# aticejiang/MLAgg-UNet

Measured on AMD Instinct MI355X. Metric: images/sec (train step) MLAgg-UNet-2D 256x256 bs10, higher is better.
Workload: dtype f32; 1 GPU; nnUNetTrainer_MLAgg_2D_dt_MS train step, AbdomenMRI-shaped 256x256x1, 14 classes, attention variant B (BASELINE.json configs[1]); batch_per_gpu=10, global_batch=10, parallelism=dp1, launch=eager, miopen=tuned find-db (mlagg-unet_amd/miopen_db), library_gemm=TunableOp table (mlagg-unet_amd/gemm_db), tuning off

## Files before the change

include/mlagg_hip.h:

```cpp
#ifndef MLAGG_HIP_H
#define MLAGG_HIP_H

#include <stddef.h>

#ifdef __cplusplus
extern "C" {
#endif

#define MLAGG_E_UNSUPPORTED (-1)
#define MLAGG_E_NULLPTR     (-2)
#define MLAGG_E_WORKSPACE   (-3)

#define MLAGG_DTYPE_F32  0
#define MLAGG_DTYPE_BF16 1
#define MLAGG_DTYPE_F16  2
#define MLAGG_DTYPE_BF16X3 3

const char *mlagg_version(void);
const char *mlagg_error_string(int code);

int mlagg_profile_kernel_count(void);
const char *mlagg_profile_kernel_name(int id);
int mlagg_profile_select(int id);
int mlagg_profile_collect(double *ms, int *counts);
// ... 45 lines not shown
                          float *dlam, float *dsubln_w, float *workspace,
                          int batch, int N, int P, int nh, float scale, void *stream);

int mlagg_dwconv3x3_fwd(const float *x, int x_stride, const float *w, const float *bias, const float *res, float *y,
                        int y_stride, float *pre, int batch, int H, int W, int C, int silu, void *stream);
size_t mlagg_dwconv3x3_bwd_workspace_floats(int batch, int H, int W, int C);
int mlagg_dwconv3x3_gated_fwd(const float *x, int x_stride, const float *w, const float *bias, const float *gate, int gate_stride, float *y,
                              int y_stride, float *pre, int batch, int H, int W, int C, void *stream);
int mlagg_dwconv3x3_gated_bwd(const float *x, int x_stride, const float *w, const float *dy, int dy_stride, const float *pre,
                              const float *gate, int gate_stride, float *dx, int dx_stride, float *dgate, int dgate_stride, float *dw,
                              float *dbias, float *workspace, int batch, int H, int W, int C, void *stream);
int mlagg_dwconv3x3_bwd(const float *x, int x_stride, const float *w, const float *dy, int dy_stride,
                        const float *pre, float *dx, int dx_stride, float *dw, float *dbias, float *workspace,
                        int batch, int H, int W, int C, int silu, void *stream);

int mlagg_linear_fwd(const float *x, int x_stride, const float *w, const float *bias, float *y, int y_stride,
                     int M, int N, int K, void *stream);
int mlagg_linear_dgrad(const float *dy, int dy_stride, const float *w, float *dx, int dx_stride, int M, int O, int I,
                       void *stream);
int mlagg_linear_lp_fwd(const float *x, int x_stride, const float *w, const float *bias, float *y, int y_stride,
                        int M, int N, int K, int dtype, void *stream);
int mlagg_linear_lp_dgrad(const float *dy, int dy_stride, const float *w, float *dx, int dx_stride, int M, int O, int I,
                          int dtype, void *stream);
size_t mlagg_linear_wgrad_workspace_floats(int M, int O, int I);
int mlagg_linear_wgrad(const float *dy, int dy_stride, const float *x, int x_stride, float *dW, float *db,
                       float *workspace, int M, int O, int I, void *stream);
int mlagg_linear_wgrad_x3(const float *dy, int dy_stride, const float *x, int x_stride, float *dW, float *db, float *workspace,
                          int M, int O, int I, void *stream);

int mlagg_flash_attn_fwd(const void *q, const void *k, const void *v, void *out, float *lse, int B, int N, int P, int nh,
                         int head_dim, float softmax_scale, int dtype, void *stream);
size_t mlagg_flash_attn_bwd_workspace_floats(int B, int N, int P, int nh, int head_dim);
int mlagg_flash_attn_bwd(const void *q, const void *k, const void *v, const void *out, const void *dout, const float *lse,
                         void *dq, float *workspace, int B, int N, int P, int nh, int head_dim, float softmax_scale,
                         int dtype, void *stream);

int mlagg_layernorm_supported(int C);
int mlagg_layernorm_fwd(const float *x, int x_stride, const float *gamma, const float *beta, float *y,
                        float *stats, int rows, int C, float eps, void *stream);
size_t mlagg_layernorm_bwd_workspace_floats(int rows, int C);
int mlagg_layernorm_bwd(const float *x, int x_stride, const float *dy, int dy_stride, const float *gamma,
                        const float *stats, float *dx, float *dgamma, float *dbeta, float *workspace,
                        int rows, int C, void *stream);
int mlagg_residual_layernorm_fwd(const float *skip, const float *branch, const float *scale, const float *gamma, const float *beta,
                                 float *xsum, float *y, float *stats, int rows, int rows_per_sample, int C, float eps, void *stream);
int mlagg_residual_layernorm_bwd(const float *xsum, const float *dy, int dy_stride, const float *dres, const float *scale,
                                 const float *gamma, const float *stats, float *dskip, float *dbranch, float *dgamma, float *dbeta,
                                 float *workspace, int rows, int rows_per_sample, int C, void *stream);

int mlagg_dwconv3d_fwd(const float *x, int x_stride, const float *w, const float *bias, float *y, int y_stride,
                       float *pre, int batch, int D, int H, int W, int C, int silu, void *stream);
size_t mlagg_dwconv3d_bwd_workspace_floats(int batch, int D, int H, int W, int C);
int mlagg_dwconv3d_bwd(const float *x, int x_stride, const float *w, const float *dy, int dy_stride, const float *pre,
                       float *dx, int dx_stride, float *dw, float *dbias, float *workspace, int batch, int D, int H,
                       int W, int C, int silu, void *stream);

int mlagg_dwconv3x3_nchw_fwd(const float *x, const float *w, const float *bias, float *y, int B, int C, int H, int W,
                             int stride, void *stream);
size_t mlagg_dwconv3x3_nchw_bwd_workspace_floats(int B, int C, int H, int W, int stride);
int mlagg_dwconv3x3_nchw_bwd(const float *x, const float *w, const float *dy, float *dx, float *dw, float *dbias,
                             float *workspace, int B, int C, int H, int W, int stride, void *stream);
int mlagg_dwconv3x3_nchw_bwd_res(const float *x, const float *w, const float *dy, const float *dres, float *dx, float *dw, float *dbias,
                                 float *workspace, int B, int C, int H, int W, int stride, void *stream);

int mlagg_cross_scan(const float *tok, int tok_stride, int blk_stride, float *seq, int B, int nscale,
                     const int *H, const int *W, int CB, int nblk, void *stream);
int mlagg_cross_merge(const float *seq, float *tok, int tok_stride, int blk_stride, int B, int nscale,
                      const int *H, const int *W, int CB, int nblk, void *stream);

int mlagg_conv1x1_supported(int O, int I, long P);
int mlagg_conv1x1_fwd(const float *x, long x_batch, const float *w, const float *bias, float *y, long y_batch, int B, int O, int I,
                      long P, void *stream);
size_t mlagg_conv1x1_wgrad_workspace_floats(int B, int O, int I, long P);
int mlagg_conv1x1_wgrad(const float *dy, long dy_batch, const float *x, long x_batch, float *dW, float *workspace, int B, int O,
                        int I, long P, void *stream);
int mlagg_conv1x1_fwd_lp(const float *x, long x_batch, const float *w, const float *bias, float *y, long y_batch, int B, int O, int I,
                         long P, int dtype, void *stream);
int mlagg_conv1x1_wgrad_lp(const float *dy, long dy_batch, const float *x, long x_batch, float *dW, float *workspace, int B, int O,
                           int I, long P, int dtype, void *stream);
int mlagg_conv1x1_fwd_ragged(const float *x, long x_batch, const float *w, const float *bias, float *y, long y_batch, int B, int O, int I,
                             int I_valid, long P, int dtype, void *stream);
int mlagg_conv1x1_fwd_acc(const float *x, long x_batch, const float *w, const float *bias, float *y, long y_batch, int B, int O, int I,
                          int I_valid, long P, int dtype, int accumulate, void *stream);

int mlagg_conv3x3_supported(int O, int I, int H, int W);
size_t mlagg_conv3x3_workspace_bytes(int O, int I);
int mlagg_conv3x3_fwd(const float *x, long x_batch, const float *w, int transposed, const float *bias, float *y, long y_batch,
                      void *workspace, int B, int O, int I, int H, int W, void *stream);
int mlagg_conv3x3x3_supported(int O, int I, int D, int H, int W);
size_t mlagg_conv3x3x3_workspace_bytes(int O, int I);
int mlagg_conv3x3x3_fwd(const float *x, long x_batch, const float *w, int transposed, const float *bias, float *y, long y_batch,
                        void *workspace, int B, int O, int I, int D, int H, int W, void *stream);
int mlagg_conv3x3_wgrad_supported(int O, int I, int H, int W);
int mlagg_conv3x3x3_wgrad_supported(int O, int I, int D, int H, int W);
size_t mlagg_conv3x3x3_wgrad_workspace_floats(int B, int O, int I, int D, int H, int W);
int mlagg_conv3x3x3_wgrad(const float *dy, long dy_batch, const float *x, long x_batch, float *dW, float *workspace, int B, int O,
                          int I, int D, int H, int W, void *stream);
size_t mlagg_conv3x3_wgrad_workspace_floats(int B, int O, int I, int H, int W);
int mlagg_conv3x3_wgrad(const float *dy, long dy_batch, const float *x, long x_batch, float *dW, float *workspace, int B, int O,
                        int I, int H, int W, void *stream);
int mlagg_conv3x3_fwd_lp(const float *x, long x_batch, const float *w, int transposed, const float *bias, float *y, long y_batch,
                         void *workspace, int B, int O, int I, int H, int W, int dtype, void *stream);
int mlagg_conv3x3_wgrad_lp(const float *dy, long dy_batch, const float *x, long x_batch, float *dW, float *workspace, int B, int O,
                           int I, int H, int W, int dtype, void *stream);

int mlagg_conv3x3_s2t_supported(int O, int I, int H, int W);
size_t mlagg_conv3x3_s2t_workspace_bytes(int O, int I);
int mlagg_conv3x3_s2t_fwd(const float *x, long x_batch, const float *w, float *y, long y_batch, void *workspace, int B, int O, int I,
                          int H, int W, int dtype, void *stream);
int mlagg_conv3x3_s2_dgrad(const float *dy, long dy_batch, long dy_chan_stride, long dy_row_stride, const float *w, float *dx,
                           long dx_batch, void *workspace, int B, int O, int I, int H, int W, int dtype, void *stream);
size_t mlagg_conv3x3_s2t_wgrad_workspace_floats(int B, int O, int I, int H, int W);
int mlagg_conv3x3_s2t_wgrad(const float *x, long x_batch, const float *dy, long dy_batch, long dy_chan_stride, long dy_row_stride,
                            float *dW, float *workspace, int B, int O, int I, int H, int W, int dtype, void *stream);

int mlagg_gelu_pool_fwd(const float *s, int s_stride, float *pooled, int batch, int H, int W, int d, int r, void *stream);
int mlagg_gelu_pool_bwd(const float *s, int s_stride, const float *dpooled, float *ds, int ds_stride, int batch, int H, int W, int d,
                        int r, void *stream);

int mlagg_gate_fwd(const float *a0, const float *a1, const float *act, int act_stride, float *out, long rows, int h,
                   void *stream);
int mlagg_gate_bwd(const float *dout, int dout_stride, const float *a0, const float *a1, const float *act, int act_stride,
                   float *da0, float *da1, float *dact, int dact_stride, long rows, int h, void *stream);

int mlagg_diff_lambda_fwd(const float *q1, const float *k1, const float *q2, const float *k2, float lambda_init, int n,
                          float *lam, float *saved_exp, void *stream);
int mlagg_diff_lambda_bwd(const float *dlam, const float *q1, const float *k1, const float *q2, const float *k2,
                          const float *saved_exp, int n, float *dq1, float *dk1, float *dq2, float *dk2, void *stream);
int mlagg_scaled_residual(const float *skip, const float *branch, const float *scale, float *out, int batch,
                          long per_sample, void *stream);
int mlagg_transpose_2d(const float *src, long src_batch_stride, float *dst, int batch, int R, int C, void *stream);
int mlagg_transpose_2d_into(const float *src, long src_batch_stride, float *dst, long dst_batch_stride, int batch, int R, int C,
                            void *stream);
int mlagg_pixel_shuffle2(const float *src, float *dst, int B, int O, int H, int W, int inverse, void *stream);
int mlagg_pixel_unshuffle2_strided(const float *src, long src_batch, float *dst, int B, int O, int H, int W, void *stream);
size_t mlagg_channel_sum_workspace_floats(int B, int C);
int mlagg_channel_sum(const float *g, float *out, float *workspace, int B, int C, long HW, void *stream);
size_t mlagg_column_sum_workspace_floats(int rows, int cols);
int mlagg_column_sum(const float *x, int x_stride, float *out, float *workspace, int rows, int cols, void *stream);

int mlagg_index_scan(const float *tok, long tok_stride, int blk_stride, const int *idx, float *seq, int B, int L, int K, int CB,
                     void *stream);
int mlagg_index_merge(const float *seq, const int *idx, float *tok, long tok_stride, int blk_stride, int B, int L, int K, int CB,
                      void *stream);
int mlagg_block_sum(const float *wide, float *out, long rows, int K, int CB, void *stream);

int mlagg_msmm_scan_supported(int d_inner, int d_state, int dt_rank, int directions, int L);
size_t mlagg_msmm_scan_state_floats(int batch, int L);
size_t mlagg_msmm_scan_fwd_workspace_floats(int batch, int L);
size_t mlagg_msmm_scan_bwd_workspace_floats(int batch, int L);
int mlagg_msmm_scan_fwd(const float *xc, const float *xdbl, const int *idx, const float *Wdt, const float *A, const float *D,
                        const float *delta_bias, float *y, float *state, float *workspace, int batch, int L, void *stream);
int mlagg_msmm_scan_bwd(const float *xc, const float *xdbl, const int *idx, const float *Wdt, const float *A, const float *D,
                        const float *delta_bias, const float *dy, const float *state, float *dxc, float *dxdbl, float *dWdt,
                        float *dA, float *dD, float *ddelta_bias, float *workspace, int batch, int L, void *stream);

int mlagg_selscan1_chunk(int B, int L, int K);
size_t mlagg_selscan1_state_floats(int B, int L, int C, int K);
int mlagg_selscan1_fwd(const float *tok, long tok_stride, const int *idx, const float *dtr, const float *Bs, const float *Cs,
                       const float *Wdt, int R, const float *A, const float *D, const float *bias, float *yk, float *state,
                       int B, int L, int C, int K, void *stream);
size_t mlagg_selscan1_bwd_workspace_floats(int B, int L, int C, int K, int R);
int mlagg_selscan1_bwd(const float *tok, long tok_stride, const int *idx, const float *dtr, const float *Bs, const float *Cs,
                       const float *Wdt, int R, const float *A, const float *D, const float *bias, const float *dout,
                       long dout_stride, const float *state, float *duk, float *ddtr, float *dBs, float *dCs, float *dparams,
                       float *workspace, int B, int L, int C, int K, void *stream);
// ... 180 lines not shown
```

mlagg-unet_amd/csrc/conv1x1.hip:

```cpp
#include <hip/hip_runtime.h>

#include <cstdlib>

#include "mlagg_hip.h"
#include "prof.h"
#include "bf16x3.h"
#include "opmode.h"
#include "internal.h"

namespace {

template <int T>
struct __attribute__((packed, aligned(4))) FVec {
    float v[T];
};

struct C1Geom {
    int B, O, I, P;
    long x_batch, y_batch;
    int I_valid;
    int accumulate;
};

using opmode::split8;
// ... 2 lines not shown
__global__ void __launch_bounds__(64)
conv1x1_fwd_kernel(const float *__restrict__ X, const float *__restrict__ W, const float *__restrict__ bias, float *__restrict__ Y,
                   C1Geom g)
{
    const int lane = threadIdx.x, col = lane & 31, kh = lane >> 5;
    const int p0 = blockIdx.x * (32 * TP), o0 = blockIdx.y * (32 * TO), b = blockIdx.z;
    f32x16 acc[TO][TP];
#pragma unroll
    for (int a = 0; a < TO; ++a)
#pragma unroll
        for (int j = 0; j < TP; ++j)
#pragma unroll
            for (int r = 0; r < 16; ++r) acc[a][j][r] = 0.f;
    const int pnat = p0 + TP * col, pc = min(pnat, g.P - TP);
    const float *xb = X + (size_t)b * g.x_batch + pc;
    const int lastrow = g.I_valid - 1;
    const float *wb[TO];
#pragma unroll
    for (int a = 0; a < TO; ++a) wb[a] = W + (size_t)min(o0 + 32 * a + col, g.O - 1) * g.I + 8 * kh;
    const int nblk = g.I / 16;
    float4 wa[2][TO][2];
    FVec<TP> xv[2][8];
    auto fetch = [&](float4 (&A)[TO][2], FVec<TP> (&Xv)[8], int blk) {
        const int kb = 16 * min(blk, nblk - 1);
#pragma unroll
        for (int t = 0; t < 8; ++t) Xv[t] = *reinterpret_cast<const FVec<TP> *>(xb + (size_t)min(kb + 8 * kh + t, lastrow) * g.P);
#pragma unroll
        for (int a = 0; a < TO; ++a) {
            A[a][0] = *reinterpret_cast<const float4 *>(wb[a] + kb);
            A[a][1] = *reinterpret_cast<const float4 *>(wb[a] + kb + 4);
        }
    };
    auto consume = [&](const float4 (&A)[TO][2], const FVec<TP> (&Xv)[8]) {
        uint4 bq[TP][3];
#pragma unroll
        for (int j = 0; j < TP; ++j) {
            const float f[8] = {Xv[0].v[j], Xv[1].v[j], Xv[2].v[j], Xv[3].v[j], Xv[4].v[j], Xv[5].v[j], Xv[6].v[j], Xv[7].v[j]};
            split8<DT>(f, bq[j]);
        }
        uint4 aq[TO][3];
#pragma unroll
        for (int a = 0; a < TO; ++a) {
            const float f[8] = {A[a][0].x, A[a][0].y, A[a][0].z, A[a][0].w, A[a][1].x, A[a][1].y, A[a][1].z, A[a][1].w};
            split8<DT>(f, aq[a]);
        }
        opmode::mfma_tiles<DT, TO, TP>(aq, bq, acc);
    };
    fetch(wa[0], xv[0], 0);
    int blk = 0;
    for (; blk + 2 <= nblk; blk += 2) {
        fetch(wa[1], xv[1], blk + 1);
        consume(wa[0], xv[0]);
        fetch(wa[0], xv[0], blk + 2);
        consume(wa[1], xv[1]);
    }
    if (blk < nblk) consume(wa[0], xv[0]);
    float *yb = Y + (size_t)b * g.y_batch + pc;
#pragma unroll
    for (int a = 0; a < TO; ++a) {
#pragma unroll
        for (int r = 0; r < 16; ++r) {
            const int o = o0 + 32 * a + (r & 3) + 8 * (r >> 2) + 4 * kh;
            if (o >= g.O) continue;
            const float bv = bias ? bias[o] : 0.f;
            float *dst = yb + (size_t)o * g.P;
            if (pc == pnat) {
                FVec<TP> v;
#pragma unroll
                for (int j = 0; j < TP; ++j) v.v[j] = acc[a][j][r] + bv;
                if (g.accumulate) {
                    const FVec<TP> old = *reinterpret_cast<const FVec<TP> *>(dst);
#pragma unroll
                    for (int j = 0; j < TP; ++j) v.v[j] += old.v[j];
                }
                *reinterpret_cast<FVec<TP> *>(dst) = v;
            } else {
#pragma unroll
                for (int j = 0; j < TP; ++j)
                    if (pc + j >= pnat) dst[j] = acc[a][j][r] + bv + (g.accumulate ? dst[j] : 0.f);
            }
        }
    }
}

struct W1Geom {
    int B, O, I, P;
    long dy_batch, x_batch;
    int slab, nslabs;
};

template <int TO, int TI, int DT>
__global__ void __launch_bounds__(64)
conv1x1_wgrad_kernel(const float *__restrict__ dY, const float *__restrict__ X, float *__restrict__ part, W1Geom g)
{
    const int lane = threadIdx.x, col = lane & 31, kh = lane >> 5;
    const int b = blockIdx.x / g.nslabs, s = blockIdx.x % g.nslabs;
    const int o0 = blockIdx.y * (32 * TO), i0 = blockIdx.z * (32 * TI);
    f32x16 acc[TO][TI];
#pragma unroll
    for (int a = 0; a < TO; ++a)
#pragma unroll
        for (int j = 0; j < TI; ++j)
#pragma unroll
            for (int r = 0; r < 16; ++r) acc[a][j][r] = 0.f;
    const int pb = s * g.slab, pe = min(pb + g.slab, g.P);
    const int nblk = (pe - pb) / 16;
    const float *ap[TO], *bp[TI];
#pragma unroll
    for (int a = 0; a < TO; ++a) ap[a] = dY + (size_t)b * g.dy_batch + (size_t)min(o0 + 32 * a + col, g.O - 1) * g.P + pb + 8 * kh;
#pragma unroll
    for (int j = 0; j < TI; ++j) bp[j] = X + (size_t)b * g.x_batch + (size_t)min(i0 + 32 * j + col, g.I - 1) * g.P + pb + 8 * kh;
    float4 av[2][TO][2], bv[2][TI][2];
    auto fetch = [&](float4 (&A)[TO][2], float4 (&Bv)[TI][2], int blk) {
        const int off = 16 * min(blk, nblk - 1);
#pragma unroll
        for (int a = 0; a < TO; ++a) {
            A[a][0] = *reinterpret_cast<const float4 *>(ap[a] + off);
            A[a][1] = *reinterpret_cast<const float4 *>(ap[a] + off + 4);
        }
#pragma unroll
        for (int j = 0; j < TI; ++j) {
            Bv[j][0] = *reinterpret_cast<const float4 *>(bp[j] + off);
            Bv[j][1] = *reinterpret_cast<const float4 *>(bp[j] + off + 4);
        }
    };
    auto consume = [&](const float4 (&A)[TO][2], const float4 (&Bv)[TI][2]) {
        uint4 bq[TI][3];
#pragma unroll
        for (int j = 0; j < TI; ++j) {
            const float f[8] = {Bv[j][0].x, Bv[j][0].y, Bv[j][0].z, Bv[j][0].w, Bv[j][1].x, Bv[j][1].y, Bv[j][1].z, Bv[j][1].w};
            split8<DT>(f, bq[j]);
        }
        uint4 aq[TO][3];
#pragma unroll
        for (int a = 0; a < TO; ++a) {
            const float f[8] = {A[a][0].x, A[a][0].y, A[a][0].z, A[a][0].w, A[a][1].x, A[a][1].y, A[a][1].z, A[a][1].w};
            split8<DT>(f, aq[a]);
        }
        opmode::mfma_tiles<DT, TO, TI>(aq, bq, acc);
    };
    if (nblk > 0) {
        fetch(av[0], bv[0], 0);
        int blk = 0;
        for (; blk + 2 <= nblk; blk += 2) {
            fetch(av[1], bv[1], blk + 1);
            consume(av[0], bv[0]);
            fetch(av[0], bv[0], blk + 2);
            consume(av[1], bv[1]);
        }
        if (blk < nblk) consume(av[0], bv[0]);
    }
    float *prow = part + (size_t)blockIdx.x * ((size_t)g.O * g.I);
#pragma unroll
    for (int a = 0; a < TO; ++a) {
#pragma unroll
        for (int j = 0; j < TI; ++j) {
            const int i = i0 + 32 * j + col;
            if (i >= g.I) continue;
#pragma unroll
            for (int r = 0; r < 16; ++r) {
                const int o = o0 + 32 * a + (r & 3) + 8 * (r >> 2) + 4 * kh;
                if (o < g.O) prow[(size_t)o * g.I + i] = acc[a][j][r];
            }
        }
    }
}

int make_wgeom(W1Geom &g, int B, int O, int I, int P, long dy_batch, long x_batch)
{
    if (B <= 0 || O <= 0 || I <= 0 || P <= 0 || (P & 15)) return MLAGG_E_UNSUPPORTED;
    if (dy_batch < (long)O * P || x_batch < (long)I * P || ((dy_batch | x_batch) & 3)) return MLAGG_E_UNSUPPORTED;
    g = W1Geom{B, O, I, P, dy_batch, x_batch, 0, 0};
    const int og = (O + 95) / 96, ig = (I + 95) / 96;
    static const int target = mlagg_internal::env_int("MLAGG_K18_WAVES", 1536, 1);
    int per_sample = (target + B * og * ig - 1) / (B * og * ig);
    if (per_sample < 1) per_sample = 1;
    int slab = (P + per_sample - 1) / per_sample;
    slab = ((slab + 15) / 16) * 16;
    if (slab < 64) slab = 64;
    g.slab = slab;
    g.nslabs = (P + slab - 1) / slab;
    if ((long)B * g.nslabs > 2147483647L || og > 65535 || ig > 65535) return MLAGG_E_UNSUPPORTED;
    return 0;
}

void pick_fwd_tile(int B, int O, int I, int P, int &to, int &tp)
{
    static const char *env = getenv("MLAGG_K18_TILE");
    if (env && env[0] >= '1' && env[0] <= '3' && env[1] == ',' && env[2] >= '1' && env[2] <= '3') {
        to = env[0] - '0';
        tp = env[2] - '0';
        if (32 * (to - 1) >= O) to = (O + 31) / 32;
    }
}

template <int TO, int TP>
void launch_fwd(const float *x, const float *w, const float *bias, float *y, const C1Geom &g, int dt, hipStream_t st)
{
    const dim3 grid((g.P + 32 * TP - 1) / (32 * TP), (g.O + 32 * TO - 1) / (32 * TO), g.B);
    if (dt == MLAGG_DTYPE_BF16)
        hipLaunchKernelGGL((conv1x1_fwd_kernel<TO, TP, MLAGG_DTYPE_BF16>), grid, dim3(64), 0, st, x, w, bias, y, g);
    else if (dt == MLAGG_DTYPE_F16)
        hipLaunchKernelGGL((conv1x1_fwd_kernel<TO, TP, MLAGG_DTYPE_F16>), grid, dim3(64), 0, st, x, w, bias, y, g);
    else
        hipLaunchKernelGGL((conv1x1_fwd_kernel<TO, TP, MLAGG_DTYPE_BF16X3>), grid, dim3(64), 0, st, x, w, bias, y, g);
}

template <int TO, int TI>
void launch_wgrad(const float *dy, const float *x, float *part, const W1Geom &g, int dt, hipStream_t st)
{
    const dim3 grid(g.B * g.nslabs, (g.O + 32 * TO - 1) / (32 * TO), (g.I + 32 * TI - 1) / (32 * TI));
    if (dt == MLAGG_DTYPE_BF16)
        hipLaunchKernelGGL((conv1x1_wgrad_kernel<TO, TI, MLAGG_DTYPE_BF16>), grid, dim3(64), 0, st, dy, x, part, g);
    else if (dt == MLAGG_DTYPE_F16)
        hipLaunchKernelGGL((conv1x1_wgrad_kernel<TO, TI, MLAGG_DTYPE_F16>), grid, dim3(64), 0, st, dy, x, part, g);
    else
        hipLaunchKernelGGL((conv1x1_wgrad_kernel<TO, TI, MLAGG_DTYPE_BF16X3>), grid, dim3(64), 0, st, dy, x, part, g);
}

}

extern "C" int mlagg_conv1x1_supported(int O, int I, long P)
{
    return O > 0 && I > 0 && (I % 16) == 0 && P >= 96 && (P % 16) == 0 && P < (1L << 30);
}

extern "C" int mlagg_conv1x1_fwd_ragged(const float *x, long x_batch, const float *w, const float *bias, float *y, long y_batch, int B,
                                        int O, int I, int I_valid, long P, int dtype, void *stream)
{
    return mlagg_conv1x1_fwd_acc(x, x_batch, w, bias, y, y_batch, B, O, I, I_valid, P, dtype, 0, stream);
}

extern "C" int mlagg_conv1x1_fwd_acc(const float *x, long x_batch, const float *w, const float *bias, float *y, long y_batch, int B,
                                     int O, int I, int I_valid, long P, int dtype, int accumulate, void *stream)
{
    if (!x || !w || !y) return MLAGG_E_NULLPTR;
    if (!opmode::valid(dtype) || I_valid <= 0 || I_valid > I) return MLAGG_E_UNSUPPORTED;
    if (B <= 0 || B > 65535 || !mlagg_conv1x1_supported(O, I, P)) return MLAGG_E_UNSUPPORTED;
    if (x_batch < (long)I_valid * P || y_batch < (long)O * P || (reinterpret_cast<uintptr_t>(w) & 15)) return MLAGG_E_UNSUPPORTED;
    C1Geom g{B, O, I, (int)P, x_batch, y_batch, I_valid, accumulate ? 1 : 0};
    hipStream_t st = static_cast<hipStream_t>(stream);
    MLAGG_TIMED(K_CONV1X1, st);
    int to = O <= 32 ? 1 : (O <= 64 ? 2 : 3), tp = O <= 64 ? 3 : 2;
    pick_fwd_tile(B, O, I, (int)P, to, tp);
    switch (to * 4 + tp) {
    case 1 * 4 + 1: launch_fwd<1, 1>(x, w, bias, y, g, dtype, st); break;
    case 1 * 4 + 2: launch_fwd<1, 2>(x, w, bias, y, g, dtype, st); break;
    case 1 * 4 + 3: launch_fwd<1, 3>(x, w, bias, y, g, dtype, st); break;
    case 2 * 4 + 1: launch_fwd<2, 1>(x, w, bias, y, g, dtype, st); break;
    case 2 * 4 + 2: launch_fwd<2, 2>(x, w, bias, y, g, dtype, st); break;
    case 2 * 4 + 3: launch_fwd<2, 3>(x, w, bias, y, g, dtype, st); break;
    case 3 * 4 + 1: launch_fwd<3, 1>(x, w, bias, y, g, dtype, st); break;
    case 3 * 4 + 2: launch_fwd<3, 2>(x, w, bias, y, g, dtype, st); break;
    default: launch_fwd<3, 3>(x, w, bias, y, g, dtype, st); break;
    }
    return (int)hipGetLastError();
}

extern "C" int mlagg_conv1x1_fwd_lp(const float *x, long x_batch, const float *w, const float *bias, float *y, long y_batch, int B,
                                    int O, int I, long P, int dtype, void *stream)
{
    return mlagg_conv1x1_fwd_ragged(x, x_batch, w, bias, y, y_batch, B, O, I, I, P, dtype, stream);
}

extern "C" int mlagg_conv1x1_fwd(const float *x, long x_batch, const float *w, const float *bias, float *y, long y_batch, int B,
                                 int O, int I, long P, void *stream)
{
    return mlagg_conv1x1_fwd_lp(x, x_batch, w, bias, y, y_batch, B, O, I, P, MLAGG_DTYPE_BF16X3, stream);
}

extern "C" size_t mlagg_conv1x1_wgrad_workspace_floats(int B, int O, int I, long P)
{
    W1Geom g;
    if (P >= (1L << 30) || make_wgeom(g, B, O, I, (int)P, (long)O * P, (long)I * P)) return 0;
    return (size_t)B * g.nslabs * O * I;
}

extern "C" int mlagg_conv1x1_wgrad_lp(const float *dy, long dy_batch, const float *x, long x_batch, float *dW, float *workspace, int B,
                                      int O, int I, long P, int dtype, void *stream)
{
    if (!dy || !x || !dW || !workspace) return MLAGG_E_NULLPTR;
    if (!opmode::valid(dtype)) return MLAGG_E_UNSUPPORTED;
    if (P >= (1L << 30)) return MLAGG_E_UNSUPPORTED;
    W1Geom g;
    if (int rc = make_wgeom(g, B, O, I, (int)P, dy_batch, x_batch)) return rc;
    if ((reinterpret_cast<uintptr_t>(dy) | reinterpret_cast<uintptr_t>(x)) & 15) return MLAGG_E_UNSUPPORTED;
    hipStream_t st = static_cast<hipStream_t>(stream);
    MLAGG_TIMED(K_CONV1X1, st);
    const int to = O > 64 ? 3 : (O + 31) / 32, ti = I > 64 ? 3 : (I + 31) / 32;
    switch (to * 4 + ti) {
    case 1 * 4 + 1: launch_wgrad<1, 1>(dy, x, workspace, g, dtype, st); break;
    case 1 * 4 + 2: launch_wgrad<1, 2>(dy, x, workspace, g, dtype, st); break;
    case 1 * 4 + 3: launch_wgrad<1, 3>(dy, x, workspace, g, dtype, st); break;
    case 2 * 4 + 1: launch_wgrad<2, 1>(dy, x, workspace, g, dtype, st); break;
    case 2 * 4 + 2: launch_wgrad<2, 2>(dy, x, workspace, g, dtype, st); break;
    case 2 * 4 + 3: launch_wgrad<2, 3>(dy, x, workspace, g, dtype, st); break;
    case 3 * 4 + 1: launch_wgrad<3, 1>(dy, x, workspace, g, dtype, st); break;
    case 3 * 4 + 2: launch_wgrad<3, 2>(dy, x, workspace, g, dtype, st); break;
    default: launch_wgrad<3, 3>(dy, x, workspace, g, dtype, st); break;
    }
    const int n = O * I;
    hipLaunchKernelGGL(mlagg_internal::column_sum_kernel<false>, dim3((n + 63) / 64), dim3(1024), 0, st, workspace, B * g.nslabs, n, n,
                       dW);
    return (int)hipGetLastError();
}

extern "C" int mlagg_conv1x1_wgrad(const float *dy, long dy_batch, const float *x, long x_batch, float *dW, float *workspace, int B,
                                   int O, int I, long P, void *stream)
{
    return mlagg_conv1x1_wgrad_lp(dy, dy_batch, x, x_batch, dW, workspace, B, O, I, P, MLAGG_DTYPE_BF16X3, stream);
}
```

mlagg-unet_amd/ops.py:

```python
import ctypes

import numpy as np
import torch

from . import _lib

_launch = _lib.launch
_stream = _lib.stream
_C = _lib.CONSTANTS


PRECISIONS = {"fp32": torch.float32, "bf16": torch.bfloat16, "fp16": torch.float16}
_LP_CODE = {torch.bfloat16: _C["MLAGG_DTYPE_BF16"], torch.float16: _C["MLAGG_DTYPE_F16"]}
import threading as _threading


class _ComputeStack(_threading.local):

    def __init__(self):
        self.stack = [torch.float32]


_COMPUTE = _ComputeStack()

# ... 1801 lines not shown
        ws = torch.empty(lib.mlagg_plane_norm_bwd_workspace_floats(B, C, hw), device=x.device, dtype=torch.float32) \
            if (dg is not None or db is not None or segmented) else None
        _launch("mlagg_plane_norm_bwd_strided", _ptr(x), _ptr(dy), dyb, _ptr(gamma), _ptr(beta), _ptr(res), _ptr(stats), _ptr(dx),
                _ptr(dres), _ptr(dg), _ptr(db), _ptr(ws), B, C, hw, act, slope, _DT_CODE[x.dtype], _DT_CODE[dy.dtype],
                0 if res is None else _DT_CODE[res.dtype])
        return dx, dg, db, dres, None, None, None, None


def plane_norm(x, gamma, beta, eps=1e-5, act=ACT_NONE, slope=0.0, res=None, out_dtype=None):
    return PlaneNormFn.apply(x, gamma, beta, res, eps, act, slope, out_dtype)


class ChannelEpilogueLpFn(torch.autograd.Function):

    @staticmethod
    def forward(ctx, x, bias, res, act, out_dtype):
        x = _require_map(x.contiguous(), "x")
        res = None if res is None else _require_map(res.contiguous(), "res", x.shape)
        B, C = x.shape[:2]
        hw = x.numel() // (B * C)
        y = torch.empty(x.shape, device=x.device, dtype=out_dtype)
        _launch("mlagg_channel_epilogue_lp_fwd", _ptr(x), _DT_CODE[x.dtype], _ptr(bias), _ptr(res),
                0 if res is None else _DT_CODE[res.dtype], _ptr(y), _DT_CODE[y.dtype], B, C, hw, int(act))
        ctx.save_for_backward(x if act == EPI_GELU else None, bias, res if act == EPI_GELU else None)
        ctx.meta = (int(act), x.dtype, None if res is None else res.dtype, tuple(x.shape))
        return y

    @staticmethod
    def backward(ctx, dy):
        x, bias, res = ctx.saved_tensors
        act, xdt, rdt, shape = ctx.meta
        dy = _require_map(dy.contiguous(), "dy", shape)
        B, C = shape[:2]
        hw = dy.numel() // (B * C)
        dx = torch.empty(shape, device=dy.device, dtype=xdt)
        db = torch.empty(C, device=dy.device, dtype=torch.float32) if bias is not None else None
        ws = (torch.empty(_lib.lib().mlagg_channel_sum_workspace_floats(B, C), device=dy.device, dtype=torch.float32)
              if bias is not None else None)
        _launch("mlagg_channel_epilogue_lp_bwd", _ptr(x), _DT_CODE[xdt], _ptr(bias), _ptr(res), 0 if res is None else _DT_CODE[res.dtype],
                _ptr(dy), _DT_CODE[dy.dtype], _ptr(dx), _DT_CODE[xdt], _ptr(db), _ptr(ws), B, C, hw, act)
        dres = None
        if rdt is not None and ctx.needs_input_grad[2]:
            src = dy if act == EPI_NONE else dx
            dres = src if src.dtype == rdt else (dx if dx.dtype == rdt else src.to(rdt))
        return dx, db, dres, None, None


def channel_epilogue_lp(x, bias=None, res=None, act=EPI_NONE, out_dtype=torch.float32):
    return ChannelEpilogueLpFn.apply(x, bias, res, act, out_dtype)


def _planes(t, name):
    _require(t, name)
    inner, want = 1, []
    for v in reversed(t.shape[1:]):
        want.append(inner)
        inner *= int(v)
    want.reverse()
    if tuple(t.stride()[1:]) != tuple(want) or t.stride(0) < inner or t.stride(0) % 4 or t.data_ptr() % 16:
        t = t.contiguous()
    return t, t.stride(0), inner // int(t.shape[1])


K18 = _os.environ.get("MLAGG_K18", "1") == "1"
K18_FWD_MIN_PIXELS = int(_os.environ.get("MLAGG_K18_FWD_MIN_PIXELS", "4096"))
K18_FWD_MIN_K = int(_os.environ.get("MLAGG_K18_FWD_MIN_K", "96"))
K18_WGRAD_MIN_PIXELS = int(_os.environ.get("MLAGG_K18_WGRAD_MIN_PIXELS", "4096"))


K18_THIN_CH = 32


def _k18_product(O, I, P, form=_DTYPE_BF16X3):
    I16 = -(-I // 16) * 16
    if not bool(_lib.lib().mlagg_conv1x1_supported(O, I16, P)):
        return False
    if form != _DTYPE_BF16X3:
        return P >= LP_K_MIN_PIXELS
    if P >= K18_FWD_MIN_PIXELS and min(O, I) <= K18_THIN_CH:
        return True
    return I == I16 and P >= K18_FWD_MIN_PIXELS and I >= K18_FWD_MIN_K


def _conv1x1_k18(x, xb, w, y, B, O, I, P, form, accumulate=False):
    if y is None:
        y = torch.empty((B, O) + tuple(x.shape[2:]), device=x.device, dtype=torch.float32)
    I16 = -(-I // 16) * 16
    if I16 != I:
        wp = torch.zeros(O, I16, device=w.device, dtype=torch.float32)
        wp[:, :I] = w
        w = wp
    _flop("K18", 2 * B * O * I * P)
    _launch("mlagg_conv1x1_fwd_acc", _ptr(x), xb, _ptr(w), None, _ptr(y), O * P, B, O, I16, I, P, form, int(accumulate))
    return y


def _conv1x1_wgrad(dy, dyb, x, B, O, I, P, form):
    dW = torch.empty(O, I, device=x.device, dtype=torch.float32)
    ws = torch.empty(_lib.lib().mlagg_conv1x1_wgrad_workspace_floats(B, O, I, P), device=x.device, dtype=torch.float32)
    _flop("K18", 2 * B * O * I * P)
    _launch("mlagg_conv1x1_wgrad_lp", _ptr(dy), dyb, _ptr(x), x.stride(0), _ptr(dW), _ptr(ws), B, O, I, P, form)
    return dW


class Conv1x1Fn(torch.autograd.Function):

    @staticmethod
    def forward(ctx, x, weight, form=_DTYPE_BF16X3, plan=None):
        x, xb, P = _planes(x, "x")
        B, I = x.shape[:2]
        O = weight.shape[0]
        plan = plan or _conv1x1_plan(O, I, P, form)
        w = _require(weight.reshape(O, I).contiguous(), "weight")
        y = _conv1x1_k18(x, xb, w, None, B, O, I, P, form) if plan[0] else _lib_conv(x, weight, 1, 0, False, form)
        ctx.save_for_backward(x, w)
        ctx.wshape, ctx.plan, ctx.form = weight.shape, plan, form
        return y

    @staticmethod
    def backward(ctx, dy):
        x, w = ctx.saved_tensors
        B, I = x.shape[:2]
        O = w.shape[0]
        dy, dyb, P = _planes(dy, "dy")
        form = ctx.form
        dx = dW = None
        if ctx.needs_input_grad[0]:
            if ctx.plan[1]:
                wt = transpose_2d(w.unsqueeze(0))[0]
                dx = _conv1x1_k18(dy, dyb, wt, None, B, I, O, P, form)
            else:
                dx = _lib_conv_bwd(dy, x, w.view(ctx.wshape), 1, 0, False, (True, False, False), form)[0]
        if ctx.needs_input_grad[1]:
            dW = _conv1x1_wgrad(dy, dyb, x, B, O, I, P, form).view(ctx.wshape)
        return dx, dW, None, None


def _conv1x1_plan(O, I, P, form):
    return ("K18" if _k18_product(O, I, P, form) else None, "K18" if _k18_product(I, O, P, form) else None, "K18")


def _pixel_shuffle2(src, B, O, H, W, inverse):
    src = _require(src.contiguous(), "src")
    dst = torch.empty((B, 4 * O, H, W) if inverse else (B, O, 2 * H, 2 * W), device=src.device, dtype=torch.float32)
    _launch("mlagg_pixel_shuffle2", _ptr(src), _ptr(dst), B, O, H, W, int(inverse))
    return dst


class ConvT2x2Fn(torch.autograd.Function):

    @staticmethod
    def forward(ctx, x, weight, form=_DTYPE_BF16X3):
        x, xb, P = _planes(x, "x")
        B, I, H, W = x.shape
        O = weight.shape[1]
        w4 = _require(weight.permute(2, 3, 1, 0).reshape(4 * O, I).contiguous(), "weight")
        z = _conv1x1_k18(x, xb, w4, None, B, 4 * O, I, P, form)
        ctx.save_for_backward(x, w4)
        ctx.form, ctx.O = form, O
        return _pixel_shuffle2(z, B, O, H, W, False)

    @staticmethod
    def backward(ctx, dy):
        x, w4 = ctx.saved_tensors
        B, I, H, W = x.shape
        O, form, P = ctx.O, ctx.form, H * W
        dy, dyb = _map_slice(dy, "dy")
        if dy.dtype != torch.float32:
            dy, dyb = dy.float(), 0
        dyu = torch.empty(B, 4 * O, H, W, device=x.device, dtype=torch.float32)
        _launch("mlagg_pixel_unshuffle2_strided", _ptr(dy), dyb, _ptr(dyu), B, O, H, W)
        dx = dW = None
        if ctx.needs_input_grad[0]:
            wt = transpose_2d(w4.unsqueeze(0))[0]
            dx = _conv1x1_k18(dyu, 4 * O * P, wt, None, B, I, 4 * O, P, form)
        if ctx.needs_input_grad[1]:
            dW = _conv1x1_wgrad(dyu, 4 * O * P, x, B, 4 * O, I, P, form).view(2, 2, O, I).permute(3, 2, 0, 1).contiguous()
        return dx, dW, None


K19 = _os.environ.get("MLAGG_K19", "1") == "1"
K19_MIN_PIXELS = int(_os.environ.get("MLAGG_K19_MIN_PIXELS", "1024"))


K19_WGRAD = _os.environ.get("MLAGG_K19_WGRAD", "1") == "1"
K19_WGRAD_MIN_PIXELS = int(_os.environ.get("MLAGG_K19_WGRAD_MIN_PIXELS", "1024"))
K19_WGRAD_MIN_CH = int(_os.environ.get("MLAGG_K19_WGRAD_MIN_CH", "48"))


def _k19_wgrad(O, I, H, W, form=_DTYPE_BF16X3):
    if form != _DTYPE_BF16X3:
        return K19_WGRAD and H * W >= LP_K_MIN_PIXELS and bool(_lib.lib().mlagg_conv3x3_wgrad_supported(O, I, H, W))
    return (K19_WGRAD and H * W >= K19_WGRAD_MIN_PIXELS and max(O, I) >= K19_WGRAD_MIN_CH and
            bool(_lib.lib().mlagg_conv3x3_wgrad_supported(O, I, H, W)))


def _k19_product(O, I, H, W, form=_DTYPE_BF16X3):
    floor = K19_MIN_PIXELS if form == _DTYPE_BF16X3 else LP_K_MIN_PIXELS
    return K19 and H * W >= floor and bool(_lib.lib().mlagg_conv3x3_supported(O, I, H, W))


def _conv3x3_plan(O, I, H, W, form):
    return tuple("K19" if on else None for on in (_k19_product(O, I, H, W, form), _k19_product(I, O, H, W, form), _k19_wgrad(O, I, H, W, form)))


def _conv3x3_k19(x, xb, w, transposed, O, I, H, W, form, out=None):
    B = x.shape[0]
    y = torch.empty(B, O, H, W, device=x.device, dtype=torch.float32) if out is None else out
    ws = torch.empty(_lib.lib().mlagg_conv3x3_workspace_bytes(O, I), device=x.device, dtype=torch.uint8)
    _flop("K19", 2 * 9 * B * O * I * H * W)
    _launch("mlagg_conv3x3_fwd_lp", _ptr(x), xb, _ptr(w), int(transposed), None, _ptr(y), y.stride(0), _ptr(ws), B, O, I, H, W, form)
    return y


class Conv3x3Fn(torch.autograd.Function):

    @staticmethod
    def forward(ctx, x, weight, form=_DTYPE_BF16X3, slot=None, plan=None):
        ctx.slot = slot
        x, xb, P = _planes(x, "x")
        B, I, H, W = x.shape
        O = weight.shape[0]
        plan = plan or _conv3x3_plan(O, I, H, W, form)
        w = _require(weight.contiguous(), "weight")
        y = _conv3x3_k19(x, xb, w, False, O, I, H, W, form) if plan[0] else _lib_conv(x, w, 1, 1, False, form)
        ctx.save_for_backward(x, w)
        ctx.plan, ctx.form = plan, form
        return y

    @staticmethod
    def backward(ctx, dy):
        x, w = ctx.saved_tensors
        B, I, H, W = x.shape
        O = w.shape[0]
        (_, dgrad, wgrad), form = ctx.plan, ctx.form
        dx = dW = None
        if ctx.needs_input_grad[0]:
            if dgrad:
                dy, dyb, _ = _planes(dy, "dy")
                out = ctx.slot.view() if ctx.slot is not None else None
                dx = _conv3x3_k19(dy, dyb, w, True, I, O, H, W, form, out)
            else:
                dx = _lib_conv_bwd(dy, x, w, 1, 1, False, (True, False, False), form)[0]
        if ctx.needs_input_grad[1]:
            if wgrad:
                lib = _lib.lib()
                dy, dyb, _ = _planes(dy, "dy")
                dW = torch.empty(O, I, 3, 3, device=x.device, dtype=torch.float32)
                ws = torch.empty(lib.mlagg_conv3x3_wgrad_workspace_floats(B, O, I, H, W), device=x.device, dtype=torch.float32)
                _flop("K19", 2 * 9 * B * O * I * H * W)
                _launch("mlagg_conv3x3_wgrad_lp", _ptr(dy), dyb, _ptr(x), x.stride(0), _ptr(dW), _ptr(ws), B, O, I, H, W, form)
            else:
                dW = _lib_conv_bwd(dy.contiguous(), x, w, 1, 1, False, (False, True, False), form)[1]
        return dx, dW, None, None, None


K19T = _os.environ.get("MLAGG_K19T", "1") == "1"
# ... 1068 lines not shown
```

Baseline: 292.5 images/sec.

## Add pre-split bf16x3 weight-image conv1x1 kernel with LDS double buffering

Adds a new 1x1 conv forward kernel whose weight operand is a precomputed bf16x3 split image. The image is staged through double-buffered shared memory across 4 waves per block, while activations are streamed via buffer loads. The Python path builds the weight images once per forward, including the transposed image, and reuses the transposed one in backward instead of transposing again. The intent is to remove per-tile weight splitting and the redundant transpose. In exchange it spends extra memory and time building the images on each step, and relies on weight_images being defined elsewhere.

```diff
diff --git a/include/mlagg_hip.h b/include/mlagg_hip.h
--- a/include/mlagg_hip.h
+++ b/include/mlagg_hip.h
@@ -151,6 +151,9 @@
                              int I_valid, long P, int dtype, void *stream);
 int mlagg_conv1x1_fwd_acc(const float *x, long x_batch, const float *w, const float *bias, float *y, long y_batch, int B, int O, int I,
                           int I_valid, long P, int dtype, int accumulate, void *stream);
+int mlagg_conv1x1_img_supported(int O, int I, long P);
+int mlagg_conv1x1_fwd_img(const float *x, long x_batch, const void *w_image, const float *bias, float *y, long y_batch, int B, int O,
+                          int I_valid, long P, int accumulate, void *stream);
 
 int mlagg_conv3x3_supported(int O, int I, int H, int W);
 size_t mlagg_conv3x3_workspace_bytes(int O, int I);
diff --git a/mlagg-unet_amd/csrc/conv1x1.hip b/mlagg-unet_amd/csrc/conv1x1.hip
--- a/mlagg-unet_amd/csrc/conv1x1.hip
+++ b/mlagg-unet_amd/csrc/conv1x1.hip
@@ -108,6 +108,123 @@
         }
     }
 }
+
+constexpr int IMG_WAVES = 4;
+
+template <int TO, int TP>
+__global__ void __launch_bounds__(64 * IMG_WAVES, 2)
+conv1x1_img_kernel(const float *__restrict__ X, const unsigned short *__restrict__ Wimg, const float *__restrict__ bias,
+                   float *__restrict__ Y, C1Geom g)
+{
+    constexpr int ROWS = 32 * TO, NTH = 64 * IMG_WAVES;
+    constexpr int HALF = 3 * ROWS * 2;
+    constexpr int STAGE = 2 * HALF;
+    constexpr int WL = (STAGE + NTH - 1) / NTH;
+    __shared__ u32x4 sW[2][STAGE];
+    const int tid = threadIdx.x, lane = tid & 63, wave = tid >> 6, col = lane & 31, kh = lane >> 5;
+    const int p0 = (blockIdx.x * IMG_WAVES + wave) * (32 * TP), o0 = blockIdx.y * ROWS, b = blockIdx.z;
+    f32x16 acc[TO][TP];
+#pragma unroll
+    for (int a = 0; a < TO; ++a)
+#pragma unroll
+        for (int j = 0; j < TP; ++j)
+#pragma unroll
+            for (int r = 0; r < 16; ++r) acc[a][j][r] = 0.f;
+    const int pnat = p0 + TP * col, pc = min(pnat, g.P - TP);
+    const int Kp = g.I;
+    const int nchunk = Kp / 32;
+    const __amdgpu_buffer_rsrc_t xrs = __builtin_amdgcn_make_buffer_rsrc(const_cast<float *>(X + (size_t)b * g.x_batch), 0,
+                                                                         4 * g.I_valid * g.P, 0x00020000);
+    const unsigned xoff = 4u * (unsigned)(8 * kh * g.P + pc);
+    unsigned wsrc[WL];
+#pragma unroll
+    for (int i = 0; i < WL; ++i) {
+        const int e = min(tid + NTH * i, STAGE - 1);
+        const int h = e & 1, row = (e >> 1) % ROWS, q = ((e >> 1) / ROWS) % 3, blk = (e >> 1) / (3 * ROWS);
+        wsrc[i] = 2u * (unsigned)(((size_t)q * g.O + min(o0 + row, g.O - 1)) * Kp + 16 * blk + 8 * h);
+    }
+    u32x4 wreg[WL];
+#define K18_WFETCH(C)                                                                                                         \
+    {                                                                                                                         \
+        const char *base_ = reinterpret_cast<const char *>(Wimg) + 64 * (size_t)min((C), nchunk - 1);                        \
+        _Pragma("unroll") for (int i_ = 0; i_ < WL; ++i_) wreg[i_] = *reinterpret_cast<const u32x4 *>(base_ + (size_t)wsrc[i_]); \
+    }
+#define K18_WSTORE(BUF)                                                                                                       \
+    {                                                                                                                         \
+        _Pragma("unroll") for (int i_ = 0; i_ < WL; ++i_) sW[(BUF)][min(tid + NTH * i_, STAGE - 1)] = wreg[i_];               \
+    }
+    FVec<TP> xv[2][8];
+    auto xfetch = [&](FVec<TP> (&Xv)[8], int blk) __attribute__((always_inline)) {
+#pragma unroll
+        for (int t = 0; t < 8; ++t) {
+            const unsigned vo = xoff + 4u * (unsigned)(16 * blk + t) * (unsigned)g.P;
+#pragma unroll
+            for (int j = 0; j < TP; ++j)
+                Xv[t].v[j] = __builtin_bit_cast(float, __builtin_amdgcn_raw_buffer_load_b32(xrs, vo, 4 * j, 0));
+        }
+    };
+    auto consume = [&](const u32x4 *wst, const FVec<TP> (&Xv)[8]) __attribute__((always_inline)) {
+        uint4 bq[TP][3];
+#pragma unroll
+        for (int j = 0; j < TP; ++j) {
+            const float f[8] = {Xv[0].v[j], Xv[1].v[j], Xv[2].v[j], Xv[3].v[j], Xv[4].v[j], Xv[5].v[j], Xv[6].v[j], Xv[7].v[j]};
+            split8<MLAGG_DTYPE_BF16X3>(f, bq[j]);
+        }
+        uint4 aq[TO][3];
+#pragma unroll
+        for (int a = 0; a < TO; ++a)
+#pragma unroll
+            for (int q = 0; q < 3; ++q) {
+                const u32x4 v = wst[(q * ROWS + 32 * a + col) * 2 + kh];
+                aq[a][q] = make_uint4(v.x, v.y, v.z, v.w);
+            }
+        opmode::mfma_tiles<MLAGG_DTYPE_BF16X3, TO, TP>(aq, bq, acc);
+    };
+    auto chunk = [&](int c, int par) __attribute__((always_inline)) {
+        K18_WFETCH(c + 1)
+        xfetch(xv[1], 2 * c + 1);
+        consume(sW[par], xv[0]);
+        xfetch(xv[0], 2 * c + 2);
+        consume(sW[par] + HALF, xv[1]);
+        K18_WSTORE(par ^ 1)
+        __syncthreads();
+    };
+    K18_WFETCH(0)
+    K18_WSTORE(0)
+    xfetch(xv[0], 0);
+    __syncthreads();
+#pragma unroll 1
+    for (int c = 0; c < nchunk; ++c) chunk(c, c & 1);
+    float *yb = Y + (size_t)b * g.y_batch + pc;
+#pragma unroll
+    for (int a = 0; a < TO; ++a) {
+#pragma unroll
+        for (int r = 0; r < 16; ++r) {
+            const int o = o0 + 32 * a + (r & 3) + 8 * (r >> 2) + 4 * kh;
+            if (o >= g.O) continue;
+            const float bv = bias ? bias[o] : 0.f;
+            float *dst = yb + (size_t)o * g.P;
+            if (pc == pnat) {
+                FVec<TP> v;
+#pragma unroll
+                for (int j = 0; j < TP; ++j) v.v[j] = acc[a][j][r] + bv;
+                if (g.accumulate) {
+                    const FVec<TP> old = *reinterpret_cast<const FVec<TP> *>(dst);
+#pragma unroll
+                    for (int j = 0; j < TP; ++j) v.v[j] += old.v[j];
+                }
+                *reinterpret_cast<FVec<TP> *>(dst) = v;
+            } else {
+#pragma unroll
+                for (int j = 0; j < TP; ++j)
+                    if (pc + j >= pnat) dst[j] = acc[a][j][r] + bv + (g.accumulate ? dst[j] : 0.f);
+            }
+        }
+    }
+}
+
+#undef K18_WFETCH
+#undef K18_WSTORE
 
 struct W1Geom {
     int B, O, I, P;
@@ -230,6 +347,14 @@
         hipLaunchKernelGGL((conv1x1_fwd_kernel<TO, TP, MLAGG_DTYPE_F16>), grid, dim3(64), 0, st, x, w, bias, y, g);
     else
         hipLaunchKernelGGL((conv1x1_fwd_kernel<TO, TP, MLAGG_DTYPE_BF16X3>), grid, dim3(64), 0, st, x, w, bias, y, g);
+}
+
+template <int TO, int TP>
+void launch_img(const float *x, const unsigned short *img, const float *bias, float *y, const C1Geom &g, hipStream_t st)
+{
+    const int groups = (g.P + 32 * TP - 1) / (32 * TP);
+    const dim3 grid((groups + IMG_WAVES - 1) / IMG_WAVES, (g.O + 32 * TO - 1) / (32 * TO), g.B);
+    hipLaunchKernelGGL((conv1x1_img_kernel<TO, TP>), grid, dim3(64 * IMG_WAVES), 0, st, x, img, bias, y, g);
 }
 
 template <int TO, int TI>
@@ -283,6 +408,35 @@
     return (int)hipGetLastError();
 }
 
+extern "C" int mlagg_conv1x1_img_supported(int O, int I, long P)
+{
+    if (O <= 0 || I <= 0 || P < 96 || (P % 16) != 0 || P >= (1L << 30)) return 0;
+    const long Ip = (I + 31) & ~31L;
+    return (Ip + 32) * P < (1L << 29) && 6L * O * Ip < (1L << 32);
+}
+
+extern "C" int mlagg_conv1x1_fwd_img(const float *x, long x_batch, const void *w_image, const float *bias, float *y, long y_batch, int B,
+                                     int O, int I_valid, long P, int accumulate, void *stream)
+{
+    if (!x || !w_image || !y) return MLAGG_E_NULLPTR;
+    if (B <= 0 || B > 65535 || !mlagg_conv1x1_img_supported(O, I_valid, P)) return MLAGG_E_UNSUPPORTED;
+    if (x_batch < (long)I_valid * P || y_batch < (long)O * P || (reinterpret_cast<uintptr_t>(w_image) & 15)) return MLAGG_E_UNSUPPORTED;
+    C1Geom g{B, O, (I_valid + 31) & ~31, (int)P, x_batch, y_batch, I_valid, accumulate ? 1 : 0};
+    hipStream_t st = static_cast<hipStream_t>(stream);
+    MLAGG_TIMED(K_CONV1X1, st);
+    const unsigned short *img = static_cast<const unsigned short *>(w_image);
+    int to = O <= 32 ? 1 : (O <= 64 ? 2 : 3), tp = O <= 64 ? 3 : 2;
+    pick_fwd_tile(B, O, I_valid, (int)P, to, tp);
+    switch (to * 4 + (tp < 2 ? 2 : tp)) {
+    case 1 * 4 + 2: launch_img<1, 2>(x, img, bias, y, g, st); break;
+    case 1 * 4 + 3: launch_img<1, 3>(x, img, bias, y, g, st); break;
+    case 2 * 4 + 2: launch_img<2, 2>(x, img, bias, y, g, st); break;
+    case 2 * 4 + 3: launch_img<2, 3>(x, img, bias, y, g, st); break;
+    default: launch_img<3, 2>(x, img, bias, y, g, st); break;
+    }
+    return (int)hipGetLastError();
+}
+
 extern "C" int mlagg_conv1x1_fwd_lp(const float *x, long x_batch, const float *w, const float *bias, float *y, long y_batch, int B,
                                     int O, int I, long P, int dtype, void *stream)
 {
diff --git a/mlagg-unet_amd/ops.py b/mlagg-unet_amd/ops.py
--- a/mlagg-unet_amd/ops.py
+++ b/mlagg-unet_amd/ops.py
@@ -1907,15 +1907,24 @@
     return I == I16 and P >= K18_FWD_MIN_PIXELS and I >= K18_FWD_MIN_K
 
 
+def _k18_operand(w, form):
+    return weight_images(w) if form == _DTYPE_BF16X3 else (w, None)
+
+
 def _conv1x1_k18(x, xb, w, y, B, O, I, P, form, accumulate=False):
     if y is None:
         y = torch.empty((B, O) + tuple(x.shape[2:]), device=x.device, dtype=torch.float32)
+    _flop("K18", 2 * B * O * I * P)
+    if form == _DTYPE_BF16X3:
+        if w.dtype != torch.uint8:
+            w = weight_images(_require(w.contiguous(), "weight", (O, I)))[0]
+        _launch("mlagg_conv1x1_fwd_img", _ptr(x), xb, _ptr(w), None, _ptr(y), O * P, B, O, I, P, int(accumulate))
+        return y
     I16 = -(-I // 16) * 16
     if I16 != I:
         wp = torch.zeros(O, I16, device=w.device, dtype=torch.float32)
         wp[:, :I] = w
         w = wp
-    _flop("K18", 2 * B * O * I * P)
     _launch("mlagg_conv1x1_fwd_acc", _ptr(x), xb, _ptr(w), None, _ptr(y), O * P, B, O, I16, I, P, form, int(accumulate))
     return y
 
@@ -1937,7 +1946,8 @@
         O = weight.shape[0]
         plan = plan or _conv1x1_plan(O, I, P, form)
         w = _require(weight.reshape(O, I).contiguous(), "weight")
-        y = _conv1x1_k18(x, xb, w, None, B, O, I, P, form) if plan[0] else _lib_conv(x, weight, 1, 0, False, form)
+        wf, ctx.wT = _k18_operand(w, form) if plan[0] or plan[1] else (None, None)
+        y = _conv1x1_k18(x, xb, wf, None, B, O, I, P, form) if plan[0] else _lib_conv(x, weight, 1, 0, False, form)
         ctx.save_for_backward(x, w)
         ctx.wshape, ctx.plan, ctx.form = weight.shape, plan, form
         return y
@@ -1952,7 +1962,7 @@
         dx = dW = None
         if ctx.needs_input_grad[0]:
             if ctx.plan[1]:
-                wt = transpose_2d(w.unsqueeze(0))[0]
+                wt = ctx.wT if ctx.wT is not None else transpose_2d(w.unsqueeze(0))[0]
                 dx = _conv1x1_k18(dy, dyb, wt, None, B, I, O, P, form)
             else:
                 dx = _lib_conv_bwd(dy, x, w.view(ctx.wshape), 1, 0, False, (True, False, False), form)[0]
@@ -1980,7 +1990,8 @@
         B, I, H, W = x.shape
         O = weight.shape[1]
         w4 = _require(weight.permute(2, 3, 1, 0).reshape(4 * O, I).contiguous(), "weight")
-        z = _conv1x1_k18(x, xb, w4, None, B, 4 * O, I, P, form)
+        wf, ctx.wT = _k18_operand(w4, form)
+        z = _conv1x1_k18(x, xb, wf, None, B, 4 * O, I, P, form)
         ctx.save_for_backward(x, w4)
         ctx.form, ctx.O = form, O
         return _pixel_shuffle2(z, B, O, H, W, False)
@@ -1997,7 +2008,7 @@
         _launch("mlagg_pixel_unshuffle2_strided", _ptr(dy), dyb, _ptr(dyu), B, O, H, W)
         dx = dW = None
         if ctx.needs_input_grad[0]:
-            wt = transpose_2d(w4.unsqueeze(0))[0]
+            wt = ctx.wT if ctx.wT is not None else transpose_2d(w4.unsqueeze(0))[0]
             dx = _conv1x1_k18(dyu, 4 * O * P, wt, None, B, I, 4 * O, P, form)
         if ctx.needs_input_grad[1]:
             dW = _conv1x1_wgrad(dyu, 4 * O * P, x, B, 4 * O, I, P, form).view(2, 2, O, I).permute(3, 2, 0, 1).contiguous()
```

Result: no change. 291.6 images/sec (-0.3%).
